# GANtastic3/MaskCycleGAN-VC

Measured on AMD Instinct MI355X. Metric: train iters/s (full G+D step), 80x64 mel bs=1, higher is better.
Workload: dtype f32

## Files before the change

maskcyclegan-vc_amd/csrc/trunk_kernels.hip:

```cpp
#include "mcvc_common.h"
#include "trace.h"
#include "launch.h"
#include "trunk.h"

#define MFMA16(a, b, c) __builtin_amdgcn_mfma_f32_16x16x4f32((a), (b), (c), 0, 0, 0)

namespace {

constexpr int kTrunkWaves = 8;
constexpr int kTrunkThreads = 64 * kTrunkWaves;

__host__ __device__ inline int trunk_doff(int KW) { return KW == 3 ? 4 : 0; }
__host__ __device__ inline int trunk_tp(int T4, int KW) { return T4 + trunk_doff(KW); }
__host__ __device__ inline int trunk_rs(int B, int T4, int KW)
{
    int rs = B * trunk_tp(T4, KW);
    if (KW == 3) { while ((rs & 7) != 4) ++rs; }
    else { while ((rs & 3) != 2) ++rs; }
    return rs;
}
__host__ __device__ inline int trunk_na(int N) { return (N + 15) >> 4; }
constexpr int kRedPitch = 80;
__host__ __device__ inline int trunk_epi_floats(int NA) { return kTrunkWaves * NA * 4 * kRedPitch + 16 * (16 * NA + 1) + 16 * 8 * 2 + 16; }

// ... 346 lines not shown
                const int f = f0 + u * kNetThreads + tid;
                if (fresh) v[u] = __builtin_bit_cast(float4, __builtin_amdgcn_raw_buffer_load_b128(rsrc, f * 16, 0, 16));
                else v[u] = (f < nf4) ? *reinterpret_cast<const float4*>(xsrc + 4ll * f) : make_float4(0.f, 0.f, 0.f, 0.f);
            }
#pragma unroll
            for (int u = 0; u < 4; ++u) {
                const int f = f0 + u * kNetThreads + tid;
                if (f < nf4) {
                    const int e = 4 * f;
                    const int r = e / T4, t = e - r * T4;
                    const int ci = r / B, b = r - ci * B;
                    float* dd = Xs + ci * RS + b * TP + DOFF + t;
                    if constexpr (KW == 3) *reinterpret_cast<float4*>(dd) = v[u];
                    else { *reinterpret_cast<float2*>(dd) = make_float2(v[u].x, v[u].y); *reinterpret_cast<float2*>(dd + 2) = make_float2(v[u].z, v[u].w); }
                }
            }
        }
    } else {
        for (int i = tid; i < Cin * B * T4; i += kNetThreads) {
            const int r = i / T4, t = i - r * T4;
            const int ci = r / B, b = r - ci * B;
            const float* q = xsrc + i;
            Xs[ci * RS + b * TP + DOFF + t] = fresh ? __hip_atomic_load(q, __ATOMIC_RELAXED, __HIP_MEMORY_SCOPE_AGENT) : *q;
        }
    }
    trunk_zero_gaps(Xs, Cin, B, TP, RS, DOFF, tid, kNetThreads);
}

template <int KW>
struct NetW { float4 wb[4][3]; };

template <int KW>
__device__ __forceinline__ void net_load_w(const TrunkLayerDesc& d, int tile, NetW<KW>& w)
{
    const int lane = threadIdx.x & 63;
    const int wave = __builtin_amdgcn_readfirstlane((int)threadIdx.x >> 6);
    const int l15 = lane & 15, kq = lane >> 4;
    const int K = d.Cin * KW;
    const int glu = (d.mode == TRUNK_IN_GLU);
    const int rows = d.rows, rows_tot = glu ? 2 * rows : rows;
    const int r0 = tile * rows;
    const int k_count = K / kNetWaves;
    const float* arow;
    if (glu) arow = (l15 < rows) ? (d.a0 + (long long)(r0 + l15) * K) : (d.a1 + (long long)(r0 + (l15 < rows_tot ? l15 - rows : 0)) * K);
    else arow = d.a0 + (long long)(r0 + (l15 < rows ? l15 : rows - 1)) * K;
    constexpr int NQ = (KW == 3) ? 3 : 2;
    constexpr int GK = 16 * NQ;
    const int sgroups = k_count / GK;
    const float* ap = arow + wave * k_count + 4 * NQ * kq;
#pragma unroll
    for (int c = 0; c < 4; ++c) {
        const float* pp = ap + (long long)(c < sgroups ? c : 0) * GK;
#pragma unroll
        for (int q = 0; q < NQ; ++q) w.wb[c][q] = *reinterpret_cast<const float4*>(pp + 4 * q);
    }
}

struct NetE { float bias[2], g0, b0, g1, b1, res; };
__device__ __forceinline__ void net_load_e(const TrunkLayerDesc& d, int B, int T4, int tile, NetE& e)
{
    const int tid = threadIdx.x;
    const int N = B * T4;
    const int glu = (d.mode == TRUNK_IN_GLU);
    const int rows = d.rows, rows_tot = glu ? 2 * rows : rows, r0 = tile * rows;
    e = NetE{{0.f, 0.f}, 0.f, 0.f, 0.f, 0.f, 0.f};
#pragma unroll
    for (int it = 0; it < 2; ++it) {
        const int el = tid + it * kNetThreads;
        if (el < rows_tot * N) {
            const int mrow = el / N;
            e.bias[it] = glu ? ((mrow < rows) ? d.bias0[r0 + mrow] : d.bias1[r0 + mrow - rows]) : d.bias0[r0 + mrow];
        }
    }
    if (tid < rows * N) {
        const int row = tid / N, col = tid - row * N, c = r0 + row;
        e.g0 = d.gamma0[c]; e.b0 = d.beta0[c];
        if (glu) { e.g1 = d.gamma1[c]; e.b1 = d.beta1[c]; }
        if (d.res) {
            const int b = col / T4, t = col - b * T4;
            e.res = __hip_atomic_load(d.res + (long long)b * d.y_sn + (long long)c * d.y_sc + t, __ATOMIC_RELAXED, __HIP_MEMORY_SCOPE_AGENT);
        }
    }
}

template <int KW, int NA>
__device__ __forceinline__ void net_tile(const TrunkLayerDesc& d, int B, int T4, float eps, int tile, const float* Xs, float* epi, bool wt,
                                         NetW<KW>& pre, const NetE& pe)
{
    const int tid = threadIdx.x;
    const int lane = tid & 63;
    const int wave = __builtin_amdgcn_readfirstlane(tid >> 6);
    const int l15 = lane & 15, kq = lane >> 4;
    constexpr int DOFF = (KW == 3) ? 4 : 0;
    const int TP = T4 + DOFF, RS = trunk_rs(B, T4, KW);
    const int N = B * T4, K = d.Cin * KW;
    const int TLP = N;
    const int glu = (d.mode == TRUNK_IN_GLU);
    const int rows = d.rows;
    const int rows_tot = glu ? 2 * rows : rows;
    const int r0 = tile * rows;
    const int Mtot = glu ? 2 * d.M : d.M;
    const int k_count = K / kNetWaves;
    const int k_begin = wave * k_count;
    const float* arow;
    {
        const int i = l15;
        if (glu) arow = (i < rows) ? (d.a0 + (long long)(r0 + i) * K) : (d.a1 + (long long)(r0 + (i < rows_tot ? i - rows : 0)) * K);
        else arow = d.a0 + (long long)(r0 + (i < rows ? i : rows - 1)) * K;
    }
    constexpr int NQ = (KW == 3) ? 3 : 2;
    constexpr int GK = 16 * NQ;
    constexpr int CH = 4;
    const int sgroups = k_count / GK;
    const float* ap = arow + k_begin + 4 * NQ * kq;
    float4 (&wb)[CH][3] = pre.wb;
    int off[NA][NQ][4];
#pragma unroll
    for (int h = 0; h < NA; ++h) {
        const int n = l15 + 16 * h;
        int xcol = B * TP, live = 0;
        if (n < N) { const int b = n / T4, t = n - b * T4; xcol = b * TP + DOFF - (KW - 1) / 2 + t; live = 1; }
#pragma unroll
        for (int q = 0; q < NQ; ++q)
#pragma unroll
            for (int j = 0; j < 4; ++j) {
                const int kr = 4 * (NQ * kq + q) + j;
                off[h][q][j] = (kr / KW) * RS + xcol + (live ? (kr % KW) : 0);
            }
    }
    f32x4 acc[NA];
#pragma unroll
    for (int h = 0; h < NA; ++h) acc[h] = f32x4{0.f, 0.f, 0.f, 0.f};
    {
        const float* xs = Xs + (k_begin / KW) * RS;
        for (int sg0 = 0; sg0 < sgroups; sg0 += CH) {
            if (sg0 > 0) {
#pragma unroll
                for (int c = 0; c < CH; ++c) {
                    const float* pp = ap + (long long)(sg0 + c < sgroups ? sg0 + c : 0) * GK;
#pragma unroll
                    for (int q = 0; q < NQ; ++q) wb[c][q] = *reinterpret_cast<const float4*>(pp + 4 * q);
                }
            }
#pragma unroll
            for (int c = 0; c < CH; ++c) {
                if (sg0 + c < sgroups) {
                    float xv[NQ][4][NA];
#pragma unroll
                    for (int q = 0; q < NQ; ++q)
#pragma unroll
                        for (int j = 0; j < 4; ++j)
#pragma unroll
                            for (int h = 0; h < NA; ++h) xv[q][j][h] = xs[off[h][q][j]];
#pragma unroll
                    for (int q = 0; q < NQ; ++q) {
                        const float av[4] = {wb[c][q].x, wb[c][q].y, wb[c][q].z, wb[c][q].w};
#pragma unroll
                        for (int j = 0; j < 4; ++j)
#pragma unroll
                            for (int h = 0; h < NA; ++h) acc[h] = MFMA16(av[j], xv[q][j][h], acc[h]);
                    }
                    __builtin_amdgcn_sched_group_barrier(0x100, NQ * 4 * NA, 0);
                    __builtin_amdgcn_sched_group_barrier(0x008, NQ * 4 * NA, 0);
                    xs += (GK / KW) * RS;
                }
            }
        }
    }
    float* red = epi;
    float* tl = epi + kNetWaves * NA * 4 * kRedPitch;
#pragma unroll
    for (int h = 0; h < NA; ++h)
#pragma unroll
        for (int r = 0; r < 4; ++r) red[((wave * NA + h) * 4 + r) * kRedPitch + lane] = acc[h][r];
    __syncthreads();
    auto row_cx = [&](int row) { return glu ? ((row < rows) ? (r0 + row) : (d.M + r0 + row - rows)) : (r0 + row); };
#pragma unroll
    for (int it = 0; it < (NA > 2 ? 2 : 1); ++it) {
        const int el = tid + it * kNetThreads;
        if (el < rows_tot * N) {
            const int mrow = el / N, col = el - mrow * N;
            const int h = col >> 4, ln = ((mrow >> 2) << 4) + (col & 15), r = mrow & 3;
            float v = 0.f;
#pragma unroll
            for (int w = 0; w < kNetWaves; ++w) v += red[((w * NA + h) * 4 + r) * kRedPitch + ln];
            v += pe.bias[it];
            tl[mrow * TLP + col] = v;
            d.conv_out[(long long)row_cx(mrow) * N + col] = v;
        }
    }
    __syncthreads();
    if (tid < rows * N) {
        const int row = tid / N, col = tid - row * N;
        const int c = r0 + row;
        const int b = col / T4, t = col - b * T4;
        const bool pow2 = (T4 & (T4 - 1)) == 0;
        auto stats_of = [&](int mrow, float& mean, float& rstd) {
            const float* p = tl + mrow * TLP + b * T4;
            float sum, q;
            if (pow2) {
                sum = p[t];
                for (int m = T4 >> 1; m >= 1; m >>= 1) sum += __shfl_xor(sum, m);
                mean = sum / (float)T4;
                const float dd = p[t] - mean;
                q = dd * dd;
                for (int m = T4 >> 1; m >= 1; m >>= 1) q += __shfl_xor(q, m);
            } else {
                sum = 0.f;
                for (int u = 0; u < T4; ++u) sum += p[u];
                mean = sum / (float)T4;
                q = 0.f;
                for (int u = 0; u < T4; ++u) { const float dd = p[u] - mean; q += dd * dd; }
            }
            rstd = 1.0f / sqrtf(q / (float)T4 + eps);
            if (t == 0) {
                float* st = d.stats + ((long long)b * Mtot + row_cx(mrow)) * 2;
                st[0] = mean; st[1] = rstd;
            }
        };
        float m0, s0;
        stats_of(row, m0, s0);
        const float z0 = (tl[row * TLP + col] - m0) * s0 * pe.g0 + pe.b0;
        float y;
        if (glu) {
            float m1, s1;
            stats_of(row + rows, m1, s1);
            const float z1 = (tl[(row + rows) * TLP + col] - m1) * s1 * pe.g1 + pe.b1;
            y = z0 * sigmoidf_(z1);
        } else {
            y = z0;
        }
        const long long yo = (long long)b * d.y_sn + (long long)c * d.y_sc + t;
        if (d.res) y += pe.res;
        if (wt) st_wt(d.y + yo, y); else d.y[yo] = y;
    }
}

template <int NA>
__global__ void __launch_bounds__(kNetThreads) trunk_fwd_net_kernel(const Twin<TrunkFwdNetArgs> tw)
{
    const TrunkFwdNetArgs& a = tw.v[blockIdx.z];
    extern __shared__ __attribute__((aligned(16))) float smem[];
    float* Xs = smem;
    float* epi = smem + a.x_floats;
    float* flag = epi + trunk_epi_floats(NA) - 16;
    const int tid = threadIdx.x;
    for (int l = 0; l < a.nlayers; ++l) {
        const TrunkLayerDesc d = a.L[l];
        const int ntiles = d.M / d.rows;
        NetW<3> w3; NetE pe;
        NetW<1>& w1 = reinterpret_cast<NetW<1>&>(w3);
        const bool mine = (int)blockIdx.x < ntiles;
        if (mine) { if (d.KW == 3) net_load_w<3>(d, blockIdx.x, w3); else net_load_w<1>(d, blockIdx.x, w1); net_load_e(d, a.B, a.T4, blockIdx.x, pe); }
        if (l > 0) {
            if (tid == 0) {
                const bool ok = wait_arrivals(a.sync + (l - 1), gridDim.x);
                if (!ok) __hip_atomic_store(a.sync + MCVC_TRUNK_SYNC_WORDS - 1, 1u + (unsigned)l, __ATOMIC_RELAXED, __HIP_MEMORY_SCOPE_AGENT);
                flag[0] = ok ? 1.f : 0.f;
            }
            asm volatile("s_waitcnt lgkmcnt(0)" ::: "memory");
            __builtin_amdgcn_s_barrier();
            if (flag[0] == 0.f) {
                const TrunkLayerDesc& dl = a.L[a.nlayers - 1];
                const int N = a.B * a.T4;
                for (int tile = blockIdx.x; tile < dl.M / dl.rows; tile += gridDim.x)
                    for (int i = tid; i < dl.rows * N; i += kNetThreads) {
                        const int row = i / N, col = i - row * N, b = col / a.T4, t = col - b * a.T4;
                        dl.y[(long long)b * dl.y_sn + (long long)(tile * dl.rows + row) * dl.y_sc + t] = __builtin_nanf("");
                    }
                return;
            }
        }
        if (d.KW == 3) net_stage_x<3>(d.x, Xs, d.Cin, a.B, a.T4, tid, l > 0); else net_stage_x<1>(d.x, Xs, d.Cin, a.B, a.T4, tid, l > 0);
        __syncthreads();
        const bool wt = (l + 1 < a.nlayers);
        for (int tile = blockIdx.x; tile < ntiles; tile += gridDim.x) {
            if (tile != (int)blockIdx.x) { if (d.KW == 3) net_load_w<3>(d, tile, w3); else net_load_w<1>(d, tile, w1); net_load_e(d, a.B, a.T4, tile, pe); }
            if (d.KW == 3) net_tile<3, NA>(d, a.B, a.T4, a.eps, tile, Xs, epi, wt, w3, pe);
            else net_tile<1, NA>(d, a.B, a.T4, a.eps, tile, Xs, epi, wt, w1, pe);
        }
        if (wt) {
            asm volatile("s_waitcnt vmcnt(0)" ::: "memory");
            __syncthreads();
            if (tid == 0 && !(a.fault_inject && l == 0 && blockIdx.x == 0))
                __hip_atomic_fetch_add(a.sync + l, 1u, __ATOMIC_RELAXED, __HIP_MEMORY_SCOPE_AGENT);
        }
    }
}

__device__ __forceinline__ void bnet_stage_pre(const TrunkBwdNetArgs& a, const TrunkBwdLayerDesc& d, float* Xs, float* rsum, int B, int T4, int tid)
{
    constexpr int DOFF = 4;
    const int TP = T4 + DOFF, RS = trunk_rs(B, T4, 3);
    const int C = d.C;
    const bool pglu = (d.pre == 2);
    const int Cx = pglu ? 2 * C : C;
    const int PB = d.pxB > 0 ? d.pxB : B;
    const float invT = 1.0f / (float)T4;
    const int E = (T4 + 3) >> 2;
    const int items = Cx * B * 4;
    const int nwg = (int)gridDim.x, me = (int)blockIdx.x;
    if (T4 == 16 && !(d.flags & TBWD_SLAB_DY) && ((reinterpret_cast<unsigned long long>(d.dy) | reinterpret_cast<unsigned long long>(d.px) |
                                                   reinterpret_cast<unsigned long long>(d.xout)) & 15ull) == 0) {
        constexpr int U = 4;
        const bool fresh = (d.flags & TBWD_DY_FRESH) != 0;
        const __amdgpu_buffer_rsrc_t rs = __builtin_amdgcn_make_buffer_rsrc(const_cast<float*>(d.dy), 0, C * B * 16 * 4, 0x00020000);
        for (int it0 = 0; it0 < items; it0 += U * kNetThreads) {
            float4 vd[U], v0[U], v1[U];
            float g0[U], b0[U], g1[U], b1[U], m0[U], r0[U], m1[U], r1[U];
#pragma unroll
            for (int u = 0; u < U; ++u) {
                const int item = it0 + u * kNetThreads + tid;
                const bool live = item < items;
                const int q4 = item & 3, row = live ? (item >> 2) : 0;
                const int cx = row / B, b = row - cx * B;
                const bool gate = pglu && cx >= C;
                const int c = gate ? cx - C : cx;
                const long long ro = ((long long)c * B + b) * 16 + q4 * 4;
                const long long po = ((long long)c * PB + b) * 16 + q4 * 4;
                vd[u] = fresh ? __builtin_bit_cast(float4, __builtin_amdgcn_raw_buffer_load_b128(rs, (int)(ro * 4), 0, 16))
                              : *reinterpret_cast<const float4*>(d.dy + ro);
                v0[u] = *reinterpret_cast<const float4*>(d.px + po);
                v1[u] = pglu ? *reinterpret_cast<const float4*>(d.px + po + (long long)C * PB * 16) : make_float4(0.f, 0.f, 0.f, 0.f);
                g0[u] = d.g0[c]; b0[u] = d.b0[c];
                g1[u] = pglu ? d.g1[c] : 0.f; b1[u] = pglu ? d.b1[c] : 0.f;
                const float* st = d.stats + (long long)b * Cx * 2;
                m0[u] = st[2 * c]; r0[u] = st[2 * c + 1];
                m1[u] = pglu ? st[2 * (c + C)] : 0.f; r1[u] = pglu ? st[2 * (c + C) + 1] : 1.f;
            }
#pragma unroll
            for (int u = 0; u < U; ++u) {
                const int item = it0 + u * kNetThreads + tid;
                const bool live = item < items;
                const int q4 = item & 3, row = live ? (item >> 2) : 0;
                const int cx = row / B, b = row - cx * B;
                const bool gate = pglu && cx >= C;
                const float dv[4] = {vd[u].x, vd[u].y, vd[u].z, vd[u].w};
                const float x0[4] = {v0[u].x, v0[u].y, v0[u].z, v0[u].w};
                const float x1[4] = {v1[u].x, v1[u].y, v1[u].z, v1[u].w};
                float dzv[4], xhv[4];
                float s1 = 0.f, s2 = 0.f;
#pragma unroll
                for (int e = 0; e < 4; ++e) {
                    const float xh0 = (x0[e] - m0[u]) * r0[u];
                    float dz, xh;
                    if (pglu) {
                        const float xh1 = (x1[e] - m1[u]) * r1[u];
                        const float sg = sigmoidf_(xh1 * g1[u] + b1[u]);
                        if (gate) { dz = dv[e] * (xh0 * g0[u] + b0[u]) * sg * (1.0f - sg); xh = xh1; }
                        else { dz = dv[e] * sg; xh = xh0; }
                    } else { dz = dv[e]; xh = xh0; }
                    dzv[e] = live ? dz : 0.f; xhv[e] = live ? xh : 0.f;
                    s1 += dzv[e]; s2 += dzv[e] * xhv[e];
                }
                s1 += __shfl_xor(s1, 1, 64); s2 += __shfl_xor(s2, 1, 64);
                s1 += __shfl_xor(s1, 2, 64); s2 += __shfl_xor(s2, 2, 64);
                if (live) {
                    const bool mine = (cx % nwg) == me;
                    const float gr = gate ? g1[u] * r1[u] : g0[u] * r0[u];
                    float o[4];
#pragma unroll
                    for (int e = 0; e < 4; ++e) o[e] = gr * (dzv[e] - s1 * invT - xhv[e] * (s2 * invT));
                    *reinterpret_cast<float4*>(Xs + cx * RS + b * TP + DOFF + q4 * 4) = make_float4(o[0], o[1], o[2], o[3]);
                    if (mine) *reinterpret_cast<float4*>(d.xout + ((long long)cx * B + b) * 16 + q4 * 4) = make_float4(o[0], o[1], o[2], o[3]);
                    if (q4 == 0 && mine) { rsum[((cx / nwg) * B + b) * 2] = s1; rsum[((cx / nwg) * B + b) * 2 + 1] = s2; }
                }
            }
        }
    } else
    for (int it0 = 0; it0 < items; it0 += kNetThreads) {
        const int item = it0 + tid;
        const bool live = item < items;
        const int q4 = item & 3, row = live ? (item >> 2) : 0;
        const int cx = row / B, b = row - cx * B;
        const bool gate = pglu && cx >= C;
        const int c = gate ? cx - C : cx;
        const float g0 = d.g0[c], b0 = d.b0[c];
        const float g1 = pglu ? d.g1[c] : 0.f, b1 = pglu ? d.b1[c] : 0.f;
        const float* st = d.stats + (long long)b * Cx * 2;
        const float m0 = st[2 * c], r0 = st[2 * c + 1];
        const float m1 = pglu ? st[2 * (c + C)] : 0.f, r1 = pglu ? st[2 * (c + C) + 1] : 1.f;
        const int t0 = q4 * E;
        const float* dyr = d.dy + ((long long)c * B + b) * T4 + t0;
        const float* x0r = d.px + ((long long)c * PB + b) * T4 + t0;
        const float* x1r = d.px + ((long long)(c + C) * PB + b) * T4 + t0;
        float vd[8], v0[8], v1[8];
#pragma unroll
        for (int e = 0; e < 8; ++e) {
            const bool ok = live && e < E && (t0 + e) < T4;
            vd[e] = ok ? ((d.flags & TBWD_DY_FRESH) ? __hip_atomic_load(dyr + e, __ATOMIC_RELAXED, __HIP_MEMORY_SCOPE_AGENT) : dyr[e]) : 0.f;
            if (ok && (d.flags & TBWD_SLAB_DY))
                for (int sl = 1; sl < a.nslab; ++sl) vd[e] += a.slabs[(long long)(sl - 1) * a.slab_stride + ((long long)c * B + b) * T4 + t0 + e];
            v0[e] = ok ? x0r[e] : 0.f; v1[e] = (ok && pglu) ? x1r[e] : 0.f;
        }
        float dzv[8], xhv[8];
        float s1 = 0.f, s2 = 0.f;
#pragma unroll
        for (int e = 0; e < 8; ++e) {
            const bool ok = e < E && (t0 + e) < T4;
            const float xh0 = (v0[e] - m0) * r0;
            float dz, xh;
            if (pglu) {
                const float xh1 = (v1[e] - m1) * r1;
                const float sg = sigmoidf_(xh1 * g1 + b1);
                if (gate) { dz = vd[e] * (xh0 * g0 + b0) * sg * (1.0f - sg); xh = xh1; }
                else { dz = vd[e] * sg; xh = xh0; }
            } else { dz = vd[e]; xh = xh0; }
            dzv[e] = ok ? dz : 0.f; xhv[e] = ok ? xh : 0.f;
            s1 += dzv[e]; s2 += dzv[e] * xhv[e];
        }
        s1 += __shfl_xor(s1, 1, 64); s2 += __shfl_xor(s2, 1, 64);
        s1 += __shfl_xor(s1, 2, 64); s2 += __shfl_xor(s2, 2, 64);
        if (live) {
            const bool mine = (cx % nwg) == me;
            const float gr = gate ? g1 * r1 : g0 * r0;
            float* xrow = Xs + cx * RS + b * TP + DOFF;
            float* od = mine ? (d.xout + ((long long)cx * B + b) * T4 + t0) : nullptr;
#pragma unroll
            for (int e = 0; e < 8; ++e) {
                if (e < E && (t0 + e) < T4) {
                    const float dxv = gr * (dzv[e] - s1 * invT - xhv[e] * (s2 * invT));
                    xrow[t0 + e] = dxv;
                    if (od) od[e] = dxv;
                }
            }
            if (q4 == 0 && mine) { rsum[((cx / nwg) * B + b) * 2] = s1; rsum[((cx / nwg) * B + b) * 2 + 1] = s2; }
        }
    }
    trunk_zero_gaps(Xs, Cx, B, TP, RS, DOFF, tid, kNetThreads);
    __syncthreads();
    for (int j = tid; j * nwg + me < Cx; j += kNetThreads) {
        const int cx = j * nwg + me;
        const bool gate = pglu && cx >= C;
        const int c = gate ? cx - C : cx;
        float dgam = 0.f, dbet = 0.f;
        for (int b = 0; b < B; ++b) { dbet += rsum[(j * B + b) * 2]; dgam += rsum[(j * B + b) * 2 + 1]; }
        float* dg = gate ? d.dg1 : d.dg0;
        float* db = gate ? d.db1 : d.db0;
        if (dg) dg[c] += dgam;
        if (db) db[c] += dbet;
    }
}

template <int NA>
__device__ __forceinline__ void bnet_tile(const TrunkBwdLayerDesc& d, int B, int T4, int tile, const float* Xs, float* epi, bool wt,
                                          NetW<3>& pre, float old)
{
    constexpr int KW = 3, DOFF = 4;
    const int tid = threadIdx.x;
    const int lane = tid & 63;
    const int wave = __builtin_amdgcn_readfirstlane(tid >> 6);
    const int l15 = lane & 15, kq = lane >> 4;
    const int TP = T4 + DOFF, RS = trunk_rs(B, T4, 3);
    const int N = B * T4;
    const int Cx = (d.pre == 2) ? 2 * d.C : d.C;
    const int K = Cx * KW;
    const int rows = d.rows, r0 = tile * rows;
    const int k_count = K / kNetWaves;
    const int k_begin = wave * k_count;
    const float* arow = d.wt + (long long)(r0 + (l15 < rows ? l15 : rows - 1)) * K;
    constexpr int NQ = 3, GK = 48, CH = 4;
    const int sgroups = k_count / GK;
    const float* ap = arow + k_begin + 4 * NQ * kq;
    float4 (&wb)[CH][3] = pre.wb;
    int off[NA][NQ][4];
#pragma unroll
    for (int h = 0; h < NA; ++h) {
        const int n = l15 + 16 * h;
        int xcol = B * TP, live = 0;
        if (n < N) { const int b = n / T4, t = n - b * T4; xcol = b * TP + DOFF - 1 + t; live = 1; }
#pragma unroll
        for (int q = 0; q < NQ; ++q)
#pragma unroll
            for (int j = 0; j < 4; ++j) {
                const int kr = 4 * (NQ * kq + q) + j;
                off[h][q][j] = (kr / KW) * RS + xcol + (live ? (kr % KW) : 0);
            }
    }
    f32x4 acc[NA];
#pragma unroll
    for (int h = 0; h < NA; ++h) acc[h] = f32x4{0.f, 0.f, 0.f, 0.f};
    {
        const float* xs = Xs + (k_begin / KW) * RS;
        for (int sg0 = 0; sg0 < sgroups; sg0 += CH) {
            if (sg0 > 0) {
#pragma unroll
                for (int c = 0; c < CH; ++c) {
                    const float* pp = ap + (long long)(sg0 + c < sgroups ? sg0 + c : 0) * GK;
#pragma unroll
                    for (int q = 0; q < NQ; ++q) wb[c][q] = *reinterpret_cast<const float4*>(pp + 4 * q);
                }
            }
#pragma unroll
            for (int c = 0; c < CH; ++c) {
                if (sg0 + c < sgroups) {
                    float xv[NQ][4][NA];
#pragma unroll
                    for (int q = 0; q < NQ; ++q)
#pragma unroll
                        for (int j = 0; j < 4; ++j)
#pragma unroll
                            for (int h = 0; h < NA; ++h) xv[q][j][h] = xs[off[h][q][j]];
#pragma unroll
                    for (int q = 0; q < NQ; ++q) {
                        const float av[4] = {wb[c][q].x, wb[c][q].y, wb[c][q].z, wb[c][q].w};
#pragma unroll
                        for (int j = 0; j < 4; ++j)
#pragma unroll
                            for (int h = 0; h < NA; ++h) acc[h] = MFMA16(av[j], xv[q][j][h], acc[h]);
                    }
                    __builtin_amdgcn_sched_group_barrier(0x100, NQ * 4 * NA, 0);
                    __builtin_amdgcn_sched_group_barrier(0x008, NQ * 4 * NA, 0);
                    xs += (GK / KW) * RS;
                }
            }
        }
    }
    float* red = epi;
#pragma unroll
    for (int h = 0; h < NA; ++h)
#pragma unroll
        for (int r = 0; r < 4; ++r) red[((wave * NA + h) * 4 + r) * kRedPitch + lane] = acc[h][r];
    __syncthreads();
    if (tid < rows * N) {
        const int mrow = tid / N, col = tid - mrow * N;
        const int h = col >> 4, ln = ((mrow >> 2) << 4) + (col & 15), r = mrow & 3;
        float v = 0.f;
#pragma unroll
        for (int w = 0; w < kNetWaves; ++w) v += red[((w * NA + h) * 4 + r) * kRedPitch + ln];
        if (d.flags & TBWD_ACCUMULATE) v += old;
        float* dst = d.out + (long long)(r0 + mrow) * N + col;
        if (wt) st_wt(dst, v); else *dst = v;
    }
}

static_assert(sizeof(Twin<TrunkBwdNetArgs>) <= 4096 && sizeof(Twin<TrunkFwdNetArgs>) <= 4096, "kernel arguments are limited to 4 KB");
template <int NA>
__global__ void __launch_bounds__(kNetThreads) trunk_bwd_net_kernel(const Twin<TrunkBwdNetArgs> tw)
{
    const TrunkBwdNetArgs& a = tw.v[blockIdx.z];
    extern __shared__ __attribute__((aligned(16))) float smem[];
    float* Xs = smem;
    float* rsum = smem + a.x_floats;
    float* epi = rsum + 16 * 8 * 2 * 2;
    float* flag = epi + kNetWaves * NA * 4 * kRedPitch;
    const int tid = threadIdx.x;
    const int N = a.B * a.T4;
    for (int l = 0; l < a.nlayers; ++l) {
        const TrunkBwdLayerDesc d = a.L[l];
        const int ntiles = d.M / d.rows;
        const int Cx = (d.pre == 2) ? 2 * d.C : d.C;
        NetW<3> w3;
        TrunkLayerDesc wd{};
        wd.a0 = d.wt; wd.Cin = Cx; wd.KW = 3; wd.M = d.M; wd.mode = TRUNK_PLAIN; wd.rows = d.rows;
        const bool mine = (int)blockIdx.x < ntiles;
        float old = 0.f;
        auto load_old = [&](int tile) {
            float v = 0.f;
            if ((d.flags & TBWD_ACCUMULATE) && tid < d.rows * N) {
                const long long idx = (long long)(tile * d.rows) * N + tid;
                v = __hip_atomic_load(d.out + idx, __ATOMIC_RELAXED, __HIP_MEMORY_SCOPE_AGENT);
                if (d.flags & TBWD_SLAB_OUT)
                    for (int sl = 1; sl < a.nslab; ++sl) v += a.slabs[(long long)(sl - 1) * a.slab_stride + idx];
            }
            return v;
        };
        if (mine) {
            net_load_w<3>(wd, blockIdx.x, w3);
            old = load_old(blockIdx.x);
        }
        if (l > 0) {
            if (tid == 0) {
                const bool ok = wait_arrivals(a.sync + (l - 1), gridDim.x);
                if (!ok) __hip_atomic_store(a.err, 0x100u + (unsigned)l, __ATOMIC_RELAXED, __HIP_MEMORY_SCOPE_AGENT);
                flag[0] = ok ? 1.f : 0.f;
            }
            asm volatile("s_waitcnt lgkmcnt(0)" ::: "memory");
            __builtin_amdgcn_s_barrier();
            if (flag[0] == 0.f) {
                const TrunkBwdLayerDesc& dl = a.L[a.nlayers - 1];
                for (int tile = blockIdx.x; tile < dl.M / dl.rows; tile += gridDim.x)
                    for (int i = tid; i < dl.rows * N; i += kNetThreads) dl.out[(long long)(tile * dl.rows) * N + i] = __builtin_nanf("");
                return;
            }
        }
        bnet_stage_pre(a, d, Xs, rsum, a.B, a.T4, tid);
        __syncthreads();
        const bool wt = (l + 1 < a.nlayers);
        for (int tile = blockIdx.x; tile < ntiles; tile += gridDim.x) {
            if (tile != (int)blockIdx.x) {
                net_load_w<3>(wd, tile, w3);
                old = load_old(tile);
            }
            bnet_tile<NA>(d, a.B, a.T4, tile, Xs, epi, wt, w3, old);
        }
        if (wt) {
            asm volatile("s_waitcnt vmcnt(0)" ::: "memory");
            __syncthreads();
            if (tid == 0 && !(a.fault_inject && l == 0 && blockIdx.x == 0))
                __hip_atomic_fetch_add(a.sync + l, 1u, __ATOMIC_RELAXED, __HIP_MEMORY_SCOPE_AGENT);
        }
    }
}

struct ZeroWordsKArgs { unsigned* p; int n; };
__global__ void zero_words_kernel(const Twin<ZeroWordsKArgs> tw)
{
    const ZeroWordsKArgs a = tw.v[blockIdx.z];
    if ((int)threadIdx.x < a.n) a.p[threadIdx.x] = 0u;
}

struct FillRowsKArgs { float* dst; const float* bias; int C; int per_row; };
__global__ void __launch_bounds__(256) fill_rows_kernel(const Twin<FillRowsKArgs> tw)
{
    const FillRowsKArgs ka_ = tw.v[blockIdx.z];
    float* __restrict__ dst = ka_.dst;
    const float* __restrict__ bias = ka_.bias;
    int C = ka_.C;
    int per_row = ka_.per_row;
    const int i = blockIdx.x * 256 + threadIdx.x;
    if (i >= C * per_row) return;
    dst[i] = bias ? bias[i / per_row] : 0.f;
}

}

int mcvc_fill_rows_launch(float* dst, const float* bias, int C, int per_row, hipStream_t s)
{
    TraceScope ts(K_ELEMENTWISE, s, 0.0, 4.0 * C * per_row);
    mcvc_launch(fill_rows_kernel, dim3((unsigned)cdiv_i(C * per_row, 256)), dim3(256), 0, s, FillRowsKArgs{dst, bias, C, per_row});
    return (int)hipGetLastError();
}

bool mcvc_trunk_applies(int Cin, int KW, int M, int B, int T4, int mode, int ksplit)
{
    if (KW != 1 && KW != 3) return false;
    if (B * T4 > 64 || T4 > 32 || B > 8) return false;
    const int K = Cin * KW;
    if (ksplit < 1 || (K % ksplit) != 0) return false;
    const int kblk = K / ksplit;
    const int gk = (KW == 3) ? 48 : 32;
    if ((kblk % (gk * kTrunkWaves)) != 0) return false;
    const int rows = (mode == TRUNK_IN_GLU) ? 8 : 16;
    if (M % rows != 0) return false;
    const long long lds = mcvc_trunk_lds_floats(Cin, KW, B, T4, ksplit);
    return lds * 4 <= 150 * 1024;
}

long long mcvc_trunk_lds_floats(int Cin, int KW, int B, int T4, int ksplit)
{
    const long long xs = (long long)(Cin / ksplit) * trunk_rs(B, T4, KW) + 4;
    const long long epi = trunk_epi_floats(trunk_na(B * T4));
    return xs > epi ? xs : epi;
}

template <int KW, int NA, bool PRE>
static int trunk_launch_p(const TrunkArgs& a, dim3 grid, size_t lds, hipStream_t s)
{
    static bool done = false;
    if (!done) {
        hipError_t e = hipFuncSetAttribute(reinterpret_cast<const void*>(trunk_layer_kernel<KW, NA, PRE>), hipFuncAttributeMaxDynamicSharedMemorySize, 160 * 1024);
        if (e != hipSuccess) return (int)e;
        done = true;
    }
    mcvc_launch((trunk_layer_kernel<KW, NA, PRE>), grid, dim3(kTrunkThreads), lds, s, a);
    return (int)hipGetLastError();
}

template <int KW, int NA>
static int trunk_launch_t(const TrunkArgs& a, dim3 grid, size_t lds, hipStream_t s)
{
    return a.pre ? trunk_launch_p<KW, NA, true>(a, grid, lds, s) : trunk_launch_p<KW, NA, false>(a, grid, lds, s);
}

template <int KW>
static int trunk_launch_k(const TrunkArgs& a, dim3 grid, size_t lds, hipStream_t s)
{
    switch (trunk_na(a.N)) {
    case 1: return trunk_launch_t<KW, 1>(a, grid, lds, s);
    case 2: return trunk_launch_t<KW, 2>(a, grid, lds, s);
    case 3: return trunk_launch_t<KW, 3>(a, grid, lds, s);
    default: return trunk_launch_t<KW, 4>(a, grid, lds, s);
    }
}

int mcvc_trunk_launch(const TrunkArgs& a, int ksplit, hipStream_t s)
{
    if (!mcvc_trunk_applies(a.Cin, a.KW, a.M, a.B, a.T4, a.mode, ksplit)) return MCVC_ERR_INVALID;
    if (ksplit > 1 && !(a.mode == TRUNK_PLAIN && (a.accumulate || a.slabs))) return MCVC_ERR_INVALID;
    if (a.slab_all && !(a.mode == TRUNK_PLAIN && a.slabs)) return MCVC_ERR_INVALID;
    if (a.pre && (a.mode != TRUNK_PLAIN || a.T4 > 32 || !a.pre_x || !a.pre_stats || !a.pre_out || (a.pre_xB > 0 && a.pre_xB < a.B))) return MCVC_ERR_INVALID;
    if (a.ky_n != 0 && !(a.ky_n == ksplit && a.ky0 >= 0 && a.ky0 < ksplit && a.mode == TRUNK_PLAIN && a.accumulate && !a.slab_all)) return MCVC_ERR_INVALID;
    const int rows = (a.mode == TRUNK_IN_GLU) ? 8 : 16;
    dim3 grid((unsigned)(a.M / rows), (unsigned)(a.ky_n > 0 ? 1 : ksplit));
    size_t lds = (size_t)mcvc_trunk_lds_floats(a.Cin, a.KW, a.B, a.T4, ksplit) * sizeof(float);
    if (a.pre) {
        const long long xs = (long long)(a.Cin / ksplit) * trunk_rs(a.B, a.T4, a.KW) + 4 + (long long)(a.Cin / ksplit) * a.B * 2;
        if ((size_t)xs * sizeof(float) > lds) lds = (size_t)xs * sizeof(float);
        if (lds > 160 * 1024) return MCVC_ERR_INVALID;
    }
    const double mt = (a.mode == TRUNK_IN_GLU) ? 2.0 * a.M : (double)a.M;
    TraceScope ts(K_TRUNK, s, 2.0 * mt * a.K * a.N, 4.0 * (mt * a.K + (double)a.Cin * a.N + 3.0 * mt * a.N));
    return a.KW == 3 ? trunk_launch_k<3>(a, grid, lds, s) : trunk_launch_k<1>(a, grid, lds, s);
}

static long long net_fwd_lds_floats(int B, int T4) { return (long long)512 * trunk_rs(B, T4, 3) + 4 + trunk_epi_floats(trunk_na(B * T4)); }
static long long net_bwd_lds_floats(int B, int T4) { return (long long)1024 * trunk_rs(B, T4, 3) + 4 + 16 * 8 * 2 * 2 + kNetWaves * trunk_na(B * T4) * 4 * kRedPitch + 16; }

static int g_trunk_passes_in_flight = 2;
static int device_cus()
{
    static const int n = [] { int dev = 0, v = 0; if (hipGetDevice(&dev) != hipSuccess || hipDeviceGetAttribute(&v, hipDeviceAttributeMultiprocessorCount, dev) != hipSuccess) v = 0; return v; }();
    return n;
}
int mcvc_trunk_set_passes_in_flight(int n) { const int was = g_trunk_passes_in_flight; if (n >= 1) g_trunk_passes_in_flight = n; return was; }
static bool trunk_residency_ok() { const int cus = device_cus(); return cus <= 0 || kNetGrid * g_trunk_passes_in_flight <= cus; }

bool mcvc_trunk_net_applies(int B, int T4)
{
    if (B < 1 || B > 8 || T4 < 1 || T4 > 32 || B * T4 > 48) return false;
    return trunk_residency_ok() && net_fwd_lds_floats(B, T4) * 4 <= 160 * 1024;
}

bool mcvc_trunk_bwd_net_applies(int B, int T4)
{
    if (B < 1 || B > 8 || T4 < 4 || T4 > 32 || B * T4 > 32) return false;
    return trunk_residency_ok() && net_bwd_lds_floats(B, T4) * 4 <= 160 * 1024;
}

static int g_trunk_fault_inject = 0;
int mcvc_trunk_set_fault_inject(int on) { const int was = g_trunk_fault_inject; g_trunk_fault_inject = on ? 1 : 0; return was; }

int mcvc_trunk_fwd_net_launch(TrunkFwdNetArgs& a, hipStream_t s)
{
    if (!mcvc_trunk_net_applies(a.B, a.T4) || a.nlayers < 1 || a.nlayers > MCVC_TRUNK_NET_LAYERS || !a.sync) return MCVC_ERR_INVALID;
    long long xmax = 0;
    double flops = 0.0, bytes = 0.0;
    const int N = a.B * a.T4;
    for (int l = 0; l < a.nlayers; ++l) {
        const TrunkLayerDesc& d = a.L[l];
        if (d.KW != 1 && d.KW != 3) return MCVC_ERR_INVALID;
        const int K = d.Cin * d.KW, gk = (d.KW == 3) ? 48 : 32;
        if (K % (gk * kNetWaves) != 0 || d.rows < 1 || d.rows > 16 || d.M % d.rows != 0) return MCVC_ERR_INVALID;
        if (d.mode == TRUNK_IN_GLU && d.rows > 8) return MCVC_ERR_INVALID;
        if (d.mode != TRUNK_IN_GLU && d.mode != TRUNK_IN) return MCVC_ERR_INVALID;
        const int rows_tot = d.mode == TRUNK_IN_GLU ? 2 * d.rows : d.rows;
        if (d.rows * N > kNetThreads || rows_tot * N > 2 * kNetThreads) return MCVC_ERR_INVALID;
        const long long x = (long long)d.Cin * trunk_rs(a.B, a.T4, d.KW) + 4;
        if (x > xmax) xmax = x;
        const double mt = (d.mode == TRUNK_IN_GLU) ? 2.0 * d.M : (double)d.M;
        flops += 2.0 * mt * K * N;
        bytes += 4.0 * (mt * K + (double)d.Cin * N + 3.0 * mt * N);
    }
    a.x_floats = (int)((xmax + 3) & ~3LL);
    a.fault_inject = g_trunk_fault_inject;
    const int NA = trunk_na(N);
    const size_t lds = ((size_t)a.x_floats + trunk_epi_floats(NA)) * sizeof(float);
    if (lds > 160 * 1024) return MCVC_ERR_INVALID;
    hipError_t e = hipSuccess;
    mcvc_launch(zero_words_kernel, dim3(1), dim3(64), 0, s, ZeroWordsKArgs{a.sync, MCVC_TRUNK_SYNC_WORDS - 1});
    TraceScope ts(K_TRUNK, s, flops, bytes);
    static bool done[4] = {false, false, false, false};
    typedef void (*KernT)(const Twin<TrunkFwdNetArgs>);
    const KernT fns[4] = {nullptr, trunk_fwd_net_kernel<1>, trunk_fwd_net_kernel<2>, trunk_fwd_net_kernel<3>};
    if (!done[NA]) {
        e = hipFuncSetAttribute(reinterpret_cast<const void*>(fns[NA]), hipFuncAttributeMaxDynamicSharedMemorySize, 160 * 1024);
        if (e != hipSuccess) return (int)e;
        done[NA] = true;
    }
    mcvc_launch(fns[NA], dim3(kNetGrid), dim3(kNetThreads), lds, s, a);
    return (int)hipGetLastError();
}

int mcvc_trunk_bwd_net_launch(TrunkBwdNetArgs& a, hipStream_t s)
{
    if (!mcvc_trunk_bwd_net_applies(a.B, a.T4) || a.nlayers < 1 || a.nlayers > MCVC_TRUNK_BWD_LAYERS || !a.sync || !a.err) return MCVC_ERR_INVALID;
    long long xmax = 0;
    double flops = 0.0, bytes = 0.0;
    const int N = a.B * a.T4;
    for (int l = 0; l < a.nlayers; ++l) {
        const TrunkBwdLayerDesc& d = a.L[l];
        const int Cx = (d.pre == 2) ? 2 * d.C : d.C;
        const int K = Cx * 3;
        if ((d.pre != 1 && d.pre != 2) || Cx > 1024 || K % (48 * kNetWaves) != 0 || d.rows < 1 || d.rows > 16 || d.M % d.rows != 0 || d.rows * N > kNetThreads ||
            (d.pxB > 0 && d.pxB < a.B))
            return MCVC_ERR_INVALID;
        const long long x = (long long)Cx * trunk_rs(a.B, a.T4, 3) + 4;
        if (x > xmax) xmax = x;
        flops += 2.0 * d.M * K * N;
        bytes += 4.0 * ((double)d.M * K + 3.0 * Cx * N + 2.0 * d.M * N);
    }
    a.x_floats = (int)((xmax + 3) & ~3LL);
    a.fault_inject = g_trunk_fault_inject;
    const bool wide = N > 16;
    const size_t lds = ((size_t)a.x_floats + 16 * 8 * 2 * 2 + kNetWaves * (wide ? 2 : 1) * 4 * kRedPitch + 16) * sizeof(float);
    if (lds > 160 * 1024) return MCVC_ERR_INVALID;
    mcvc_launch(zero_words_kernel, dim3(1), dim3(64), 0, s, ZeroWordsKArgs{a.sync, MCVC_TRUNK_SYNC_WORDS - 1});
    TraceScope ts(K_TRUNK, s, flops, bytes);
    static bool done[2] = {false, false};
    if (!done[wide]) {
        const void* fn = wide ? reinterpret_cast<const void*>(trunk_bwd_net_kernel<2>) : reinterpret_cast<const void*>(trunk_bwd_net_kernel<1>);
        hipError_t e = hipFuncSetAttribute(fn, hipFuncAttributeMaxDynamicSharedMemorySize, 160 * 1024);
        if (e != hipSuccess) return (int)e;
        done[wide] = true;
    }
    if (wide) mcvc_launch(trunk_bwd_net_kernel<2>, dim3(kNetGrid), dim3(kNetThreads), lds, s, a);
    else mcvc_launch(trunk_bwd_net_kernel<1>, dim3(kNetGrid), dim3(kNetThreads), lds, s, a);
    return (int)hipGetLastError();
}
```

Before: 178.6.

## Fuse next-layer norm/GLU backward into trunk bwd tile epilogue and alias LDS

```diff
diff --git a/maskcyclegan-vc_amd/csrc/trunk_kernels.hip b/maskcyclegan-vc_amd/csrc/trunk_kernels.hip
--- a/maskcyclegan-vc_amd/csrc/trunk_kernels.hip
+++ b/maskcyclegan-vc_amd/csrc/trunk_kernels.hip
@@ -672,7 +672,7 @@
     const int nwg = (int)gridDim.x, me = (int)blockIdx.x;
     if (T4 == 16 && !(d.flags & TBWD_SLAB_DY) && ((reinterpret_cast<unsigned long long>(d.dy) | reinterpret_cast<unsigned long long>(d.px) |
                                                    reinterpret_cast<unsigned long long>(d.xout)) & 15ull) == 0) {
-        constexpr int U = 4;
+        constexpr int U = 2;
         const bool fresh = (d.flags & TBWD_DY_FRESH) != 0;
         const __amdgpu_buffer_rsrc_t rs = __builtin_amdgcn_make_buffer_rsrc(const_cast<float*>(d.dy), 0, C * B * 16 * 4, 0x00020000);
         for (int it0 = 0; it0 < items; it0 += U * kNetThreads) {
@@ -812,26 +812,65 @@
     }
 }
 
-template <int NA>
-__device__ __forceinline__ void bnet_tile(const TrunkBwdLayerDesc& d, int B, int T4, int tile, const float* Xs, float* epi, bool wt,
-                                          NetW<3>& pre, float old)
+struct BnetP { float g0, b0, g1, b1, m0, r0, m1, r1; float v0[4], v1[4]; float dgo, dbo; };
+__device__ __forceinline__ void bnet_load_p(const TrunkBwdLayerDesc& nd, int B, int T4, int row0, int rows, BnetP& p)
+{
+    const int C = nd.C;
+    const bool pglu = (nd.pre == 2);
+    const int Cx = pglu ? 2 * C : C;
+    const int PB = nd.pxB > 0 ? nd.pxB : B;
+    const int E = (T4 + 3) >> 2;
+    const int items = (pglu ? 2 * rows : rows) * B * 4;
+    const int item = threadIdx.x;
+    const bool live = item < items;
+    const int q4 = item & 3, row = live ? (item >> 2) : 0;
+    const int xr = row / B, b = row - xr * B;
+    const int c = row0 + (xr >= rows ? xr - rows : xr);
+    p.g0 = live ? nd.g0[c] : 0.f; p.b0 = live ? nd.b0[c] : 0.f;
+    p.g1 = (live && pglu) ? nd.g1[c] : 0.f; p.b1 = (live && pglu) ? nd.b1[c] : 0.f;
+    const float* st = nd.stats + (long long)b * Cx * 2;
+    p.m0 = live ? st[2 * c] : 0.f; p.r0 = live ? st[2 * c + 1] : 0.f;
+    p.m1 = (live && pglu) ? st[2 * (c + C)] : 0.f; p.r1 = (live && pglu) ? st[2 * (c + C) + 1] : 1.f;
+    const int t0 = q4 * E;
+    const float* x0r = nd.px + ((long long)c * PB + b) * T4 + t0;
+    const float* x1r = nd.px + ((long long)(c + C) * PB + b) * T4 + t0;
+#pragma unroll
+    for (int e = 0; e < 4; ++e) {
+        const bool ok = live && e < E && (t0 + e) < T4;
+        p.v0[e] = ok ? x0r[e] : 0.f; p.v1[e] = (ok && pglu) ? x1r[e] : 0.f;
+    }
+    p.dgo = 0.f; p.dbo = 0.f;
+    if ((int)threadIdx.x < (pglu ? 2 * rows : rows)) {
+        const int xr2 = threadIdx.x;
+        const bool gate2 = pglu && xr2 >= rows;
+        const int c2 = row0 + (gate2 ? xr2 - rows : xr2);
+        const float* dg = gate2 ? nd.dg1 : nd.dg0;
+        const float* db = gate2 ? nd.db1 : nd.db0;
+        if (dg) p.dgo = dg[c2];
+        if (db) p.dbo = db[c2];
+    }
+}
+
+template <typename WSG>
+__device__ __forceinline__ void bnet_load_w(WSG wsg, int stot, NetW<3>& w)
+{
+#pragma unroll
+    for (int c = 0; c < 4; ++c) {
+        const float* pp = wsg(c < stot ? c : 0);
+#pragma unroll
+        for (int q = 0; q < 3; ++q) w.wb[c][q] = *reinterpret_cast<const float4*>(pp + 4 * q);
+    }
+}
+
+template <int NA, typename WSG>
+__device__ __forceinline__ void bnet_mma(f32x4 (&acc)[NA], NetW<3>& pre, WSG wsg, const float* xs, int s0, int s1, int stot, int B, int T4)
 {
     constexpr int KW = 3, DOFF = 4;
-    const int tid = threadIdx.x;
-    const int lane = tid & 63;
-    const int wave = __builtin_amdgcn_readfirstlane(tid >> 6);
+    const int lane = threadIdx.x & 63;
     const int l15 = lane & 15, kq = lane >> 4;
     const int TP = T4 + DOFF, RS = trunk_rs(B, T4, 3);
     const int N = B * T4;
-    const int Cx = (d.pre == 2) ? 2 * d.C : d.C;
-    const int K = Cx * KW;
-    const int rows = d.rows, r0 = tile * rows;
-    const int k_count = K / kNetWaves;
-    const int k_begin = wave * k_count;
-    const float* arow = d.wt + (long long)(r0 + (l15 < rows ? l15 : rows - 1)) * K;
     constexpr int NQ = 3, GK = 48, CH = 4;
-    const int sgroups = k_count / GK;
-    const float* ap = arow + k_begin + 4 * NQ * kq;
     float4 (&wb)[CH][3] = pre.wb;
     int off[NA][NQ][4];
 #pragma unroll
@@ -847,46 +886,51 @@
                 off[h][q][j] = (kr / KW) * RS + xcol + (live ? (kr % KW) : 0);
             }
     }
-    f32x4 acc[NA];
-#pragma unroll
-    for (int h = 0; h < NA; ++h) acc[h] = f32x4{0.f, 0.f, 0.f, 0.f};
-    {
-        const float* xs = Xs + (k_begin / KW) * RS;
-        for (int sg0 = 0; sg0 < sgroups; sg0 += CH) {
-            if (sg0 > 0) {
-#pragma unroll
-                for (int c = 0; c < CH; ++c) {
-                    const float* pp = ap + (long long)(sg0 + c < sgroups ? sg0 + c : 0) * GK;
+    for (int sg0 = s0 & ~(CH - 1); sg0 < s1; sg0 += CH) {
+#pragma unroll
+        for (int c = 0; c < CH; ++c) {
+            if (sg0 + c >= s0 && sg0 + c < s1) {
+                float xv[NQ][4][NA];
+#pragma unroll
+                for (int q = 0; q < NQ; ++q)
+#pragma unroll
+                    for (int j = 0; j < 4; ++j)
+#pragma unroll
+                        for (int h = 0; h < NA; ++h) xv[q][j][h] = xs[off[h][q][j]];
+#pragma unroll
+                for (int q = 0; q < NQ; ++q) {
+                    const float av[4] = {wb[c][q].x, wb[c][q].y, wb[c][q].z, wb[c][q].w};
+#pragma unroll
+                    for (int j = 0; j < 4; ++j)
+#pragma unroll
+                        for (int h = 0; h < NA; ++h) acc[h] = MFMA16(av[j], xv[q][j][h], acc[h]);
+                }
+                __builtin_amdgcn_sched_group_barrier(0x100, NQ * 4 * NA, 0);
+                __builtin_amdgcn_sched_group_barrier(0x008, NQ * 4 * NA, 0);
+                if (sg0 + c + CH < stot) {
+                    const float* pp = wsg(sg0 + c + CH);
 #pragma unroll
                     for (int q = 0; q < NQ; ++q) wb[c][q] = *reinterpret_cast<const float4*>(pp + 4 * q);
                 }
-            }
-#pragma unroll
-            for (int c = 0; c < CH; ++c) {
-                if (sg0 + c < sgroups) {
-                    float xv[NQ][4][NA];
-#pragma unroll
-                    for (int q = 0; q < NQ; ++q)
-#pragma unroll
-                        for (int j = 0; j < 4; ++j)
-#pragma unroll
-                            for (int h = 0; h < NA; ++h) xv[q][j][h] = xs[off[h][q][j]];
-#pragma unroll
-                    for (int q = 0; q < NQ; ++q) {
-                        const float av[4] = {wb[c][q].x, wb[c][q].y, wb[c][q].z, wb[c][q].w};
-#pragma unroll
-                        for (int j = 0; j < 4; ++j)
-#pragma unroll
-                            for (int h = 0; h < NA; ++h) acc[h] = MFMA16(av[j], xv[q][j][h], acc[h]);
-                    }
-                    __builtin_amdgcn_sched_group_barrier(0x100, NQ * 4 * NA, 0);
-                    __builtin_amdgcn_sched_group_barrier(0x008, NQ * 4 * NA, 0);
-                    xs += (GK / KW) * RS;
-                }
-            }
-        }
-    }
+                __builtin_amdgcn_sched_group_barrier(0x020, NQ, 0);
+                xs += (GK / KW) * RS;
+            }
+        }
+    }
+}
+
+template <int NA>
+__device__ __forceinline__ void bnet_epilogue(const TrunkBwdLayerDesc& d, const TrunkBwdLayerDesc& nd, bool emit, const BnetP& p, int B, int T4, int tile,
+                                              const f32x4 (&acc)[NA], float* epi, float* tl, float* rs, bool wt, float old)
+{
+    const int tid = threadIdx.x;
+    const int lane = tid & 63;
+    const int wave = __builtin_amdgcn_readfirstlane(tid >> 6);
+    const int N = B * T4;
+    const int rows = d.rows, r0 = tile * rows;
     float* red = epi;
+    asm volatile("s_waitcnt lgkmcnt(0)" ::: "memory");
+    __builtin_amdgcn_s_barrier();
 #pragma unroll
     for (int h = 0; h < NA; ++h)
 #pragma unroll
@@ -901,6 +945,86 @@
         if (d.flags & TBWD_ACCUMULATE) v += old;
         float* dst = d.out + (long long)(r0 + mrow) * N + col;
         if (wt) st_wt(dst, v); else *dst = v;
+        tl[tid] = v;
+    }
+    if (!emit) return;
+    __syncthreads();
+    const int C = nd.C;
+    const bool pglu = (nd.pre == 2);
+    const int E = (T4 + 3) >> 2;
+    const float invT = 1.0f / (float)T4;
+    const int xrows = pglu ? 2 * rows : rows;
+    const int items = xrows * B * 4;
+    {
+        const int item = tid;
+        const bool live = item < items;
+        const int q4 = item & 3, row = live ? (item >> 2) : 0;
+        const int xr = row / B, b = row - xr * B;
+        const bool gate = pglu && xr >= rows;
+        const int lr = gate ? xr - rows : xr;
+        const int cx = r0 + lr + (gate ? C : 0);
+        const int t0 = q4 * E;
+        const float* dyr = tl + (lr * B + b) * T4 + t0;
+        const int PB = nd.pxB > 0 ? nd.pxB : B;
+        const int cc = r0 + lr;
+        const float* x0r = nd.px + ((long long)cc * PB + b) * T4 + t0;
+        const float* x1r = nd.px + ((long long)(cc + C) * PB + b) * T4 + t0;
+        const float g0 = p.g0, b0 = p.b0, g1 = p.g1, b1 = p.b1, m0 = p.m0, r0_ = p.r0, m1 = p.m1, r1 = p.r1;
+        float dzv[8], xhv[8];
+        float s1 = 0.f, s2 = 0.f;
+#pragma unroll
+        for (int e = 0; e < 8; ++e) {
+            dzv[e] = 0.f; xhv[e] = 0.f;
+            if (e < E) {
+                const bool ok = (t0 + e) < T4;
+                const float vd = (live && ok) ? dyr[e] : 0.f;
+                float pv0, pv1;
+                if (e < 4) { pv0 = p.v0[e]; pv1 = p.v1[e]; }
+                else {
+                    pv0 = (live && ok) ? x0r[e] : 0.f; pv1 = (live && ok && pglu) ? x1r[e] : 0.f;
+                }
+                const float xh0 = (pv0 - m0) * r0_;
+                float dz, xh;
+                if (pglu) {
+                    const float xh1 = (pv1 - m1) * r1;
+                    const float sg = sigmoidf_(xh1 * g1 + b1);
+                    if (gate) { dz = vd * (xh0 * g0 + b0) * sg * (1.0f - sg); xh = xh1; }
+                    else { dz = vd * sg; xh = xh0; }
+                } else { dz = vd; xh = xh0; }
+                dzv[e] = ok ? dz : 0.f; xhv[e] = ok ? xh : 0.f;
+            }
+            s1 += dzv[e]; s2 += dzv[e] * xhv[e];
+        }
+        s1 += __shfl_xor(s1, 1, 64); s2 += __shfl_xor(s2, 1, 64);
+        s1 += __shfl_xor(s1, 2, 64); s2 += __shfl_xor(s2, 2, 64);
+        if (live) {
+            const float gr = gate ? g1 * r1 : g0 * r0_;
+            float* od = nd.xout + ((long long)cx * B + b) * T4 + t0;
+#pragma unroll
+            for (int e = 0; e < 8; ++e) {
+                if (e < E && (t0 + e) < T4) {
+                    const float dxv = gr * (dzv[e] - s1 * invT - xhv[e] * (s2 * invT));
+                    st_wt(od + e, dxv);
+                }
+            }
+            if (q4 == 0) {
+                int ri = item >> 2;
+                asm volatile("" : "+v"(ri));
+                rs[ri * 2] = s1; rs[ri * 2 + 1] = s2;
+            }
+        }
+    }
+    __syncthreads();
+    if (tid < xrows) {
+        const int xr = tid;
+        const bool gate = pglu && xr >= rows;
+        const int c = r0 + (gate ? xr - rows : xr);
+        float dgam = 0.f, dbet = 0.f;
+        for (int b = 0; b < B; ++b) { dbet += rs[(xr * B + b) * 2]; dgam += rs[(xr * B + b) * 2 + 1]; }
+        float* dg = gate ? nd.dg1 : nd.dg0;
+        float* db = gate ? nd.db1 : nd.db0;
+        if (dg) dg[c] = p.dgo + dgam;
+        if (db) db[c] = p.dbo + dbet;
     }
 }
 
@@ -912,32 +1036,37 @@
     extern __shared__ __attribute__((aligned(16))) float smem[];
     float* Xs = smem;
     float* rsum = smem + a.x_floats;
-    float* epi = rsum + 16 * 8 * 2 * 2;
-    float* flag = epi + kNetWaves * NA * 4 * kRedPitch;
+    float* flag = rsum + 16 * 8 * 2 * 2;
+    float* tl = flag + 16;
+    float* epi = Xs;
     const int tid = threadIdx.x;
+    const int lane = tid & 63;
+    const int wave = __builtin_amdgcn_readfirstlane(tid >> 6);
     const int N = a.B * a.T4;
+    const int RS = trunk_rs(a.B, a.T4, 3);
     for (int l = 0; l < a.nlayers; ++l) {
         const TrunkBwdLayerDesc d = a.L[l];
-        const int ntiles = d.M / d.rows;
+        const bool wt = (l + 1 < a.nlayers);
+        const TrunkBwdLayerDesc nd = a.L[wt ? l + 1 : l];
         const int Cx = (d.pre == 2) ? 2 * d.C : d.C;
+        const int K = Cx * 3;
+        const int sT = Cx / 128;
         NetW<3> w3;
-        TrunkLayerDesc wd{};
-        wd.a0 = d.wt; wd.Cin = Cx; wd.KW = 3; wd.M = d.M; wd.mode = TRUNK_PLAIN; wd.rows = d.rows;
-        const bool mine = (int)blockIdx.x < ntiles;
+        BnetP p;
+        const int tile = blockIdx.x;
+        const bool mine = tile < d.M / d.rows;
         float old = 0.f;
-        auto load_old = [&](int tile) {
-            float v = 0.f;
+        const float* ap = d.wt + (long long)(tile * d.rows + ((lane & 15) < d.rows ? (lane & 15) : d.rows - 1)) * K + wave * (K / kNetWaves) + 12 * (lane >> 4);
+        auto wsg = [&](int sg) { return ap + (long long)sg * 48; };
+        if (mine) {
+            bnet_load_w(wsg, sT, w3);
             if ((d.flags & TBWD_ACCUMULATE) && tid < d.rows * N) {
                 const long long idx = (long long)(tile * d.rows) * N + tid;
-                v = __hip_atomic_load(d.out + idx, __ATOMIC_RELAXED, __HIP_MEMORY_SCOPE_AGENT);
+                old = __hip_atomic_load(d.out + idx, __ATOMIC_RELAXED, __HIP_MEMORY_SCOPE_AGENT);
                 if (d.flags & TBWD_SLAB_OUT)
-                    for (int sl = 1; sl < a.nslab; ++sl) v += a.slabs[(long long)(sl - 1) * a.slab_stride + idx];
-            }
-            return v;
-        };
-        if (mine) {
-            net_load_w<3>(wd, blockIdx.x, w3);
-            old = load_old(blockIdx.x);
+                    for (int sl = 1; sl < a.nslab; ++sl) old += a.slabs[(long long)(sl - 1) * a.slab_stride + idx];
+            }
+            if (wt && l > 0) bnet_load_p(nd, a.B, a.T4, tile * d.rows, d.rows, p);
         }
         if (l > 0) {
             if (tid == 0) {
@@ -949,20 +1078,22 @@
             __builtin_amdgcn_s_barrier();
             if (flag[0] == 0.f) {
                 const TrunkBwdLayerDesc& dl = a.L[a.nlayers - 1];
-                for (int tile = blockIdx.x; tile < dl.M / dl.rows; tile += gridDim.x)
-                    for (int i = tid; i < dl.rows * N; i += kNetThreads) dl.out[(long long)(tile * dl.rows) * N + i] = __builtin_nanf("");
+                for (int t = blockIdx.x; t < dl.M / dl.rows; t += gridDim.x)
+                    for (int i = tid; i < dl.rows * N; i += kNetThreads) dl.out[(long long)(t * dl.rows) * N + i] = __builtin_nanf("");
                 return;
             }
-        }
-        bnet_stage_pre(a, d, Xs, rsum, a.B, a.T4, tid);
+            net_stage_x<3>(d.xout, Xs, Cx, a.B, a.T4, tid, true);
+        } else {
+            bnet_stage_pre(a, d, Xs, rsum, a.B, a.T4, tid);
+            if (mine && wt) bnet_load_p(nd, a.B, a.T4, tile * d.rows, d.rows, p);
+        }
         __syncthreads();
-        const bool wt = (l + 1 < a.nlayers);
-        for (int tile = blockIdx.x; tile < ntiles; tile += gridDim.x) {
-            if (tile != (int)blockIdx.x) {
-                net_load_w<3>(wd, tile, w3);
-                old = load_old(tile);
-            }
-            bnet_tile<NA>(d, a.B, a.T4, tile, Xs, epi, wt, w3, old);
+        if (mine) {
+            f32x4 acc[NA];
+#pragma unroll
+            for (int h = 0; h < NA; ++h) acc[h] = f32x4{0.f, 0.f, 0.f, 0.f};
+            bnet_mma<NA>(acc, w3, wsg, Xs + wave * (Cx / kNetWaves) * RS, 0, sT, sT, a.B, a.T4);
+            bnet_epilogue<NA>(d, nd, wt, p, a.B, a.T4, tile, acc, epi, tl, rsum, wt, old);
         }
         if (wt) {
             asm volatile("s_waitcnt vmcnt(0)" ::: "memory");
@@ -1075,7 +1206,9 @@
 }
 
 static long long net_fwd_lds_floats(int B, int T4) { return (long long)512 * trunk_rs(B, T4, 3) + 4 + trunk_epi_floats(trunk_na(B * T4)); }
-static long long net_bwd_lds_floats(int B, int T4) { return (long long)1024 * trunk_rs(B, T4, 3) + 4 + 16 * 8 * 2 * 2 + kNetWaves * trunk_na(B * T4) * 4 * kRedPitch + 16; }
+static const long long kNetBwdLdsBytes = 160 * 1024;
+static const long long kNetBwdEpiFloats = 16 * 8 * 2 * 2 + 16 + 512;
+static long long net_bwd_lds_floats(int B, int T4) { return (long long)1024 * trunk_rs(B, T4, 3) + 4 + kNetBwdEpiFloats; }
 
 static int g_trunk_passes_in_flight = 2;
 static int device_cus()
@@ -1095,7 +1228,7 @@
 bool mcvc_trunk_bwd_net_applies(int B, int T4)
 {
     if (B < 1 || B > 8 || T4 < 4 || T4 > 32 || B * T4 > 32) return false;
-    return trunk_residency_ok() && net_bwd_lds_floats(B, T4) * 4 <= 160 * 1024;
+    return trunk_residency_ok() && net_bwd_lds_floats(B, T4) * 4 <= kNetBwdLdsBytes;
 }
 
 static int g_trunk_fault_inject = 0;
@@ -1148,6 +1281,8 @@
     long long xmax = 0;
     double flops = 0.0, bytes = 0.0;
     const int N = a.B * a.T4;
+    const int RS = trunk_rs(a.B, a.T4, 3);
+    const bool wide = N > 16;
     for (int l = 0; l < a.nlayers; ++l) {
         const TrunkBwdLayerDesc& d = a.L[l];
         const int Cx = (d.pre == 2) ? 2 * d.C : d.C;
@@ -1155,16 +1290,20 @@
         if ((d.pre != 1 && d.pre != 2) || Cx > 1024 || K % (48 * kNetWaves) != 0 || d.rows < 1 || d.rows > 16 || d.M % d.rows != 0 || d.rows * N > kNetThreads ||
             (d.pxB > 0 && d.pxB < a.B))
             return MCVC_ERR_INVALID;
-        const long long x = (long long)Cx * trunk_rs(a.B, a.T4, 3) + 4;
+        if (d.M / d.rows > kNetGrid) return MCVC_ERR_INVALID;
+        if (l + 1 < a.nlayers && (a.L[l + 1].dy != d.out || a.L[l + 1].C != d.M || !a.L[l + 1].xout)) return MCVC_ERR_INVALID;
+        if (l + 1 < a.nlayers && (a.L[l + 1].pre == 2 ? 2 : 1) * d.rows * a.B * 4 > kNetThreads) return MCVC_ERR_INVALID;
+        const long long x = (long long)Cx * RS + 4;
         if (x > xmax) xmax = x;
         flops += 2.0 * d.M * K * N;
         bytes += 4.0 * ((double)d.M * K + 3.0 * Cx * N + 2.0 * d.M * N);
     }
+    const long long red = (long long)kNetWaves * (wide ? 2 : 1) * 4 * kRedPitch;
+    if (xmax < red) xmax = red;
     a.x_floats = (int)((xmax + 3) & ~3LL);
     a.fault_inject = g_trunk_fault_inject;
-    const bool wide = N > 16;
-    const size_t lds = ((size_t)a.x_floats + 16 * 8 * 2 * 2 + kNetWaves * (wide ? 2 : 1) * 4 * kRedPitch + 16) * sizeof(float);
-    if (lds > 160 * 1024) return MCVC_ERR_INVALID;
+    const size_t lds = ((size_t)a.x_floats + (size_t)kNetBwdEpiFloats) * sizeof(float);
+    if (lds > (size_t)kNetBwdLdsBytes) return MCVC_ERR_INVALID;
     mcvc_launch(zero_words_kernel, dim3(1), dim3(64), 0, s, ZeroWordsKArgs{a.sync, MCVC_TRUNK_SYNC_WORDS - 1});
     TraceScope ts(K_TRUNK, s, flops, bytes);
     static bool done[2] = {false, false};
```

After: 180.1, median of 6. About the same (+0.8%).
